# zhouxian/FluidLab

Hardware: AMD Instinct MI355X
Metric: MPM substeps/sec (fwd+bwd), 128^3 grid / 200k particles (higher is better)
Workload: dtype f32; 1 GPU; water block 128^3 grid, 200k particles (BASELINE configs[1] inputs), fwd+bwd, evolving (rolling window); nc_start=34727, nc_end=99195, parallelism=1 env, 1 GPU

## Files before the change

fluidlab_amd/csrc/fe_engine.hip:

```cpp
#include <hip/hip_runtime.h>

#include <algorithm>
#include <cstdio>
#include <cstdlib>
#include <cstring>
#include <string>
#include <vector>

#include "../../include/fluidengine.h"
#include "../../include/fluidengine_ext.h"
#include "fe_math.h"
#include "fe_grid_launch.h"

static_assert(sizeof(fe_real) == 4, "the HIP engine is fp32 (macros.py:207-211)");

#define FR_WORDS 25
#define GR_WORDS 24

template <typename T>
struct Plane {
    char* base; unsigned off;
    __host__ __device__ __forceinline__ T& operator[](int s) const { return *(T*)(base + (size_t)(off + (unsigned)s * (unsigned)sizeof(T))); }
    __host__ __device__ __forceinline__ T* ptr() const { return (T*)(base + (size_t)off); }
};
// ... 499 lines not shown
template <int NPL>
__device__ __forceinline__ void slab_store(float4* slab, int item, int l, float4 v, int wt) {
    float4* base = slab + (size_t)item * SLAB_N;
    if (NPL == 4) { if (wt) wt_store16(base, (unsigned)l * 16u, v); else base[l] = v; }
    else {
        const u32x3 u = {__float_as_uint(v.x), __float_as_uint(v.y), __float_as_uint(v.z)};
        if (wt) __builtin_amdgcn_raw_buffer_store_b96(u, wt_rsrc(base), l * 12, 0, 16);
        else __builtin_amdgcn_raw_buffer_store_b96(u, wt_rsrc(base), l * 12, 0, 0);
    }
}
__device__ __forceinline__ int tile_region(int t) { return (t + 3) >> 2; }
template <int NPL, bool SHELL_ONLY = false, bool FG = false>
__device__ __forceinline__ void tile_handover(const SimP& S, float4* slab, int item, float* acc, const GridStore& GS, const TileO& to,
                                              int nbr_entry, int l, float4 v, int wt, int& fg_d) {
    asm volatile("" : "+v"(l));
    const int tx = l >> 6, ty = (l >> 3) & 7, tz = l & 7;
    const int reg = tile_region(tx) * 9 + tile_region(ty) * 3 + tile_region(tz);
    const int e = __shfl(nbr_entry, reg, 64);
    const bool inner = ((unsigned)(tx - 1) < (unsigned)SLAB_T) & ((unsigned)(ty - 1) < (unsigned)SLAB_T) & ((unsigned)(tz - 1) < (unsigned)SLAB_T);
    if (inner) {
        if (!SHELL_ONLY) slab_store<NPL>(slab, item, ((tx - 1) * SLAB_T + (ty - 1)) * SLAB_T + (tz - 1), v, wt);
    } else if (e >= 0 && (v.x != 0.f || v.y != 0.f || v.z != 0.f || v.w != 0.f)) {
        float* dst = acc + cell_addr(to.ox + tx, to.oy + ty, to.oz + tz, S.nb);
        unsafeAtomicAdd(dst, v.x); unsafeAtomicAdd(dst + S.ncell, v.y); unsafeAtomicAdd(dst + 2 * S.ncell, v.z);
        if (NPL > 3) unsafeAtomicAdd(dst + 3 * S.ncell, v.w);
        if (FG) fg_d |= 1 << reg; else GS.dirty[e] = GS.stamp;
    }
}
template <int NPL, bool SHELL_ONLY = false>
__device__ __forceinline__ void tile_handover(const SimP& S, float4* slab, int item, float* acc, const GridStore& GS, const TileO& to,
                                              int nbr_entry, int l, float4 v, int wt) {
    int none = 0;
    tile_handover<NPL, SHELL_ONLY, false>(S, slab, item, acc, GS, to, nbr_entry, l, v, wt, none);
}

#ifndef FE_LEAN_QUADS
#define FE_LEAN_QUADS 0
#endif
__device__ __forceinline__ bool stencil_on_shell(int lb) {
    const int bx = lb >> 6, by = (lb >> 3) & 7, bz = lb & 7;
    return (bx == 0) | (bx == 5) | (by == 0) | (by == 5) | (bz == 0) | (bz == 5);
}
template <int NPL, bool FG = false>
__device__ __forceinline__ void quad_handover(const SimP& S, const int* acc, float inv_p, float inv_m, float4* slab, int item, float* accg,
                                              const GridStore& GS, const TileO& to, int nbr_entry, bool wshell, int wt, int& fg_d) {
    int lane = threadIdx.x & 63;
    asm volatile("" : "+v"(lane));
#if !FE_LEAN_QUADS
    for (int k = 0; k < TILE_N / 64; k++) {
        const int l = lane + 64 * k;
        tile_handover<NPL, false, FG>(S, slab, item, accg, GS, to, nbr_entry, l, make_float4((float)acc[l] * inv_p, (float)acc[TILE_N + l] * inv_p, (float)acc[2 * TILE_N + l] * inv_p, NPL > 3 ? (float)acc[3 * TILE_N + l] * inv_m : 0.f), wt, fg_d);
    }
    return;
#endif
#pragma unroll
    for (int k = 0; k < 4; k++) {
        const int l6 = lane + 64 * k;
        if (k < 3 || l6 < SLAB_N) {
            const int tx = l6 / 36, r = l6 - 36 * tx, ty = r / 6, tz = r - 6 * ty;
            const int l = ((tx + 1) * TILE_T + ty + 1) * TILE_T + tz + 1;
            const float4 v = make_float4((float)acc[l] * inv_p, (float)acc[TILE_N + l] * inv_p, (float)acc[2 * TILE_N + l] * inv_p, NPL > 3 ? (float)acc[3 * TILE_N + l] * inv_m : 0.f);
            slab_store<NPL>(slab, item, l6, v, wt);
        }
    }
    if (wshell) {
#pragma unroll 2
        for (int k = 0; k < TILE_N / 64; k++) {
            const int l = lane + 64 * k;
            const int tx = l >> 6, ty = (l >> 3) & 7, tz = l & 7;
            const bool inner = ((unsigned)(tx - 1) < (unsigned)SLAB_T) & ((unsigned)(ty - 1) < (unsigned)SLAB_T) & ((unsigned)(tz - 1) < (unsigned)SLAB_T);
            float4 v = make_float4(0.f, 0.f, 0.f, 0.f);
            if (!inner) v = make_float4((float)acc[l] * inv_p, (float)acc[TILE_N + l] * inv_p, (float)acc[2 * TILE_N + l] * inv_p, NPL > 3 ? (float)acc[3 * TILE_N + l] * inv_m : 0.f);
            tile_handover<NPL, true, FG>(S, slab, item, accg, GS, to, nbr_entry, l, v, wt, fg_d);
        }
    }
}
template <int NPL>
__device__ __forceinline__ void quad_handover(const SimP& S, const int* acc, float inv_p, float inv_m, float4* slab, int item, float* accg,
                                              const GridStore& GS, const TileO& to, int nbr_entry, bool wshell, int wt) {
    int none = 0;
    quad_handover<NPL, false>(S, acc, inv_p, inv_m, slab, item, accg, GS, to, nbr_entry, wshell, wt, none);
}

struct GridW {
    float* g_in; float4* slab; int ncell; int* frame_slow; int* blk_flag; int* blk_list; int* blk_count; int* err; int* slow;
    const FgDev* fg; float4* g_out;
};

__device__ __forceinline__ void carry_F(const FrameV& cur, const FrameV& nxt, m3& F) {
    if (nxt.iso == 1 && cur.iso != 1) { const float c = fe_cbrt_pos(m3_det(F)); F = m3_zero(); F.a[0][0] = F.a[1][1] = F.a[2][2] = c; }
}
__device__ __forceinline__ void unused_particle_fwd(const SimP& S, const FrameV& cur, const FrameV& nxt, int s, int pid,
                                                    const int* __restrict__ pool_idx, const AgentP& agent, const InjectP& inj, int f) {
    PState p;
    load_xvC(cur, s, p);
    load_F(cur, s, p.F);
    int used_next = 0;
    if (inj.on) {
        int j = pool_idx[pid] - inj.act_id;
        if (j >= 0 && j < inj.flux) {
            const EffP& e = agent.e[agent.inj];
            const float* rv = e.random_vector + ((size_t)inj.row * e.flux + j) * 3;
            float q[4] = {e.quat[f * 4], e.quat[f * 4 + 1], e.quat[f * 4 + 2], e.quat[f * 4 + 3]};
            float ip[3], iv[3];
            quat_rotate(e.inject_p, q, ip);
            quat_rotate(e.inject_v, q, iv);
            float vnorm = sqrtf(e.inject_v[0] * e.inject_v[0] + e.inject_v[1] * e.inject_v[1] + e.inject_v[2] * e.inject_v[2]);
#pragma unroll
            for (int d = 0; d < 3; d++) {
                float offset = (rv[d] * 2.f - 1.f) * e.radius;
                p.x[d] = offset + e.pos[f * 3 + d] + ip[d];
                p.v[d] = e.randomize_inject_v ? iv[d] + (rv[d] * 2.f - 1.f) * vnorm * 2.0f : iv[d];
            }
            used_next = 1;
        }
    }
    store_xvC(nxt, s, p.x, p.v, p.C);
    carry_F(cur, nxt, p.F);
    store_F(nxt, s, p.F);
    pstore(nxt, nxt.used, s, used_next);
}

__device__ __forceinline__ bool collector_takes(const SimP& S, const FrameV& cur, const FrameV& nxt, int s, const float4* __restrict__ info, const AgentP& agent) {
    if (agent.collector_mat >= 0 && load_info(S, info, s).mat != agent.collector_mat) return false;
    PState p;
    load_xvC(cur, s, p);
    if (!boundary_is_out(*agent.collector, p.x)) return false;
    load_F(cur, s, p.F);
    const float nowhere[3] = {-100.f, -100.f, -100.f};
    store_xvC(nxt, s, nowhere, p.v, p.C);
    carry_F(cur, nxt, p.F);
    store_F(nxt, s, p.F);
    cur.used[s] = 0; nxt.used[s] = 0;
    return true;
}

struct P2GPrep { Stencil st; float mv[3]; m3 affine; float m; bool inside; };

struct P2GRaw { PState p; PInfo info; };
__device__ __forceinline__ void p2g_load(const SimP& S, const FrameV& cur, int s, const float4* __restrict__ info_, P2GRaw& r) {
    load_xvC(cur, s, r.p);
    load_F(cur, s, r.p.F);
    r.info = load_info(S, info_, s);
}
template <bool WRITE, bool GENERAL>
__device__ __forceinline__ void p2g_compute(const SimP& S, const FrameV& nxt, int s, const P2GRaw& r, const GridW& G, P2GPrep& q, bool primary = true) {
    const PState& p = r.p;
    const PInfo& info = r.info;
    Constitutive k;
    constitutive_eval_t<GENERAL>(p.C, p.F, S.dt, info.mu, info.lam, info.mass, info.cls, S.stress_scale, k);
    if (WRITE && primary) store_F_used(nxt, s, k.Fnew, 1);
    stencil_make(p.x, S.inv_dx, q.st);
    q.inside = stencil_inside(q.st, S.n);
    if (!q.inside && primary) atomicAdd(G.err, 1);
    q.m = info.mass;
    q.affine = k.affine;
#pragma unroll
    for (int a = 0; a < 3; a++)
        q.mv[a] = q.m * p.v[a] - S.dx * (k.affine.a[a][0] * q.st.fx[0] + k.affine.a[a][1] * q.st.fx[1] + k.affine.a[a][2] * q.st.fx[2]);
}
template <bool WRITE, bool GENERAL>
__device__ __forceinline__ void p2g_prepare(const SimP& S, const FrameV& cur, const FrameV& nxt, int s,
                                            const float4* __restrict__ info_, const GridW& G, P2GPrep& q) {
    P2GRaw r;
    p2g_load(S, cur, s, info_, r);
    p2g_compute<WRITE, GENERAL>(S, nxt, s, r, G, q);
// ... 198 lines not shown
        for (int kk = 0; kk < 3; kk++) {
            const float weight = wij * st.w[kk][2];
            const float4 gv = g_out[cell_addr(st.base[0] + i, st.base[1] + j, st.base[2] + kk, S.nb)];
            const float gw[3] = {weight * gv.x, weight * gv.y, weight * gv.z};
#pragma unroll
            for (int a = 0; a < 3; a++) {
                if (kk == 0) T[a] = gw[a];
                else { T[a] = T[a] + gw[a]; Tz[a] = kk == 1 ? gw[a] : __builtin_fmaf(2.f, gw[a], Tz[a]); }
            }
        }
        const float fi = (float)i, fj = (float)j;
#pragma unroll
        for (int a = 0; a < 3; a++) {
            nv[a] = nv[a] + T[a];
            M.a[a][0] = __builtin_fmaf(fi, T[a], M.a[a][0]); M.a[a][1] = __builtin_fmaf(fj, T[a], M.a[a][1]); M.a[a][2] = M.a[a][2] + Tz[a];
        }
    }
#pragma unroll
    for (int a = 0; a < 3; a++)
#pragma unroll
        for (int b = 0; b < 3; b++) nC.a[a][b] = c4 * __builtin_fmaf(-st.fx[b], nv[a], M.a[a][b]);
}
template <bool TILE, bool ALIAS, bool ROLLED = false>
__device__ __forceinline__ void g2p_gather(const SimP& S, int lb, const Stencil& st, const float4* __restrict__ g_out, int tofs, float nv[3], m3& nC) {
    if (!TILE) { g2p_gather_global<true, ALIAS ? FE_SLOW_UNR : 1>(S, st, g_out, nv, nC); return; }
    const float* gt = ALIAS ? (const float*)s_acc : s_gtile;
    nv[0] = nv[1] = nv[2] = 0.f;
    const float c4 = 4.f * S.inv_dx;
    m3 M = m3_zero();
#pragma unroll ROLLED ? 1 : 9
    for (int ij = 0; ij < 9; ij++) {
        const int i = ij / 3, j = ij - 3 * i;
        const float wij = STW(st, i, 0) * STW(st, j, 1);
        float T[3] = {0.f, 0.f, 0.f}, Tz[3] = {0.f, 0.f, 0.f};
#pragma unroll
        for (int kk = 0; kk < 3; kk++) {
            const float weight = wij * st.w[kk][2];
            float g0, g1, g2;
            if (TILE) {
                const int l = tofs + lb + (i * TILE_T + j) * TILE_T + kk;
                g0 = gt[l]; g1 = gt[TILE_N + l]; g2 = gt[2 * TILE_N + l];
            } else {
                float4 gv = g_out[cell_addr(st.base[0] + i, st.base[1] + j, st.base[2] + kk, S.nb)];
                g0 = gv.x; g1 = gv.y; g2 = gv.z;
            }
            const float gw[3] = {weight * g0, weight * g1, weight * g2};
#pragma unroll
            for (int a = 0; a < 3; a++) { T[a] += gw[a]; if (kk > 0) Tz[a] += (float)kk * gw[a]; }
        }
#pragma unroll
        for (int a = 0; a < 3; a++) {
            nv[a] += T[a];
            M.a[a][0] += (float)i * T[a]; M.a[a][1] += (float)j * T[a]; M.a[a][2] += Tz[a];
        }
    }
#pragma unroll
    for (int a = 0; a < 3; a++)
#pragma unroll
        for (int b = 0; b < 3; b++) nC.a[a][b] = c4 * (M.a[a][b] - st.fx[b] * nv[a]);
}
template <int NIT, typename LD, typename ST>
__device__ __forceinline__ void tile_nodes_n(int t0, int nth, LD&& ld, ST&& st) {
    float4 v[NIT];
#pragma unroll
    for (int it = 0; it < NIT; it++) v[it] = ld(t0 + it * nth);
#pragma unroll
    for (int it = 0; it < NIT; it++) st(t0 + it * nth, v[it]);
}
template <bool QUADS = true, int MAXIT = 8, typename LD, typename ST>
__device__ __forceinline__ void tile_nodes(int t0, int nth, LD&& ld, ST&& st) {
    if (nth == WG) tile_nodes_n<2>(t0, nth, ld, st);
    else if (!QUADS || nth == HALF) {
        if constexpr (MAXIT >= 4) tile_nodes_n<4>(t0, nth, ld, st);
        else { tile_nodes_n<2>(t0, nth, ld, st); tile_nodes_n<2>(t0 + 2 * nth, nth, ld, st); }
    } else {
        if constexpr (MAXIT >= 8) tile_nodes_n<8>(t0, nth, ld, st);
        else if constexpr (MAXIT >= 4) { tile_nodes_n<4>(t0, nth, ld, st); tile_nodes_n<4>(t0 + 4 * nth, nth, ld, st); }
        else { for (int r = 0; r < 4; r++) tile_nodes_n<2>(t0 + 2 * r * nth, nth, ld, st); }
    }
}
__device__ __forceinline__ float4 tile_node_load(const TileO& to, const SimP& S, const float4* __restrict__ src, int l) {
    int i, j, k;
    const bool ok = tile_node(to, l, S.n, i, j, k);
    const float4 v = src[ok ? cell_addr(i, j, k, S.nb) : 0];
    return make_float4(ok ? v.x : 0.f, ok ? v.y : 0.f, ok ? v.z : 0.f, ok ? v.w : 0.f);
}
template <bool ALIAS = false>
__device__ __forceinline__ void load_tile3(const TileO& to, const SimP& S, const float4* __restrict__ src, const PairCtx& pc, int tofs_alias = 0) {
    if (!pc.live) return;
    float* gt = ALIAS ? (float*)s_acc : s_gtile;
    const int tofs = ALIAS ? tofs_alias : pc.ti * 3 * TILE_N;
    tile_nodes<ALIAS>(pc.t0, pc.nth, [&](int l) { return tile_node_load(to, S, src, l); },
                      [&](int l, const float4 v) { gt[tofs + l] = v.x; gt[tofs + TILE_N + l] = v.y; gt[tofs + 2 * TILE_N + l] = v.z; });
}

struct FuseP { float* fr_prev; const float4* g_out; int* slow; int* blk_count_prev; };
template <bool WRITE, bool GENERAL, bool FUSED = false, bool FG = false>
__device__ __forceinline__ void p2g_body(SimP S, float* fr_cur, float* fr_next, TableP T,
                                            const int* __restrict__ pool_idx, GridW G, AgentP agent, InjectP inj, int act, int f,
                                            GridStore GS, int fiso, FuseP FU = FuseP{nullptr, nullptr, nullptr, nullptr}) {
    const UnitAsk ask0 = unit_ask(T, blockIdx.x);
    const int n_slots = T.meta[5];
    HEAD_END(T.units_cap);
    if (!WRITE && GS.cap > 0 && GS.flag[f]) return;
    const int tid = threadIdx.x;
    if (WRITE && blockIdx.x == 0 && tid == 0 && act) {
        for (int i = 0; i < agent.n; i++) effector_move(agent.e[i], f);
    }
    if (FG) {
        if (blockIdx.x == 0 && tid == 0 && GS.cap > 0) __hip_atomic_store(GS.flag + f, 1, __ATOMIC_RELAXED, __HIP_MEMORY_SCOPE_AGENT);
        fg_begin(G.fg);
    }
    if (FUSED && blockIdx.x == 0 && tid == 0) *FU.blk_count_prev = 0;
    FrameV cur = frame_view(fr_cur, S.Np, 0, (!GENERAL && (fiso & 1)) ? 1 : 0);
    FrameV curw = frame_view(fr_cur, S.Np, 0);
    FrameV prev = frame_view(FUSED ? FU.fr_prev : fr_cur, S.Np);
    FrameV nxt = frame_view(fr_next, S.Np, S.wt & 1, (!GENERAL && (fiso & 2)) ? 1 : 0);
    const int slab_wt = FG ? 1 : (S.wt & 1);
    TL(S, 0);
    Unit un = unit_take(ask0);
    bool prev_quad = false;
    for (int wg = blockIdx.x; FG || wg < n_slots; wg += gridDim.x) {
        if (FG || wg != (int)blockIdx.x) un = unit_load(T, wg);
        if (FG && wg >= n_slots) break;
        if (un.a.z == -2) continue;
        if (un.a.z >= 0) {
            const PairCtx pc = unit_ctx(un);
            unit_enter(pc.quad, prev_quad);
            const int4 it = pc.it;
            const TileO to = tile_origin(it.x);
            const int aofs = pc.ti * 4 * TILE_N;
            int fg_t = 0, fg_d = 0;
            TL(S, 1);
            const int nbr_entry = neighbour_entry(T.blk_slot, S.nb, it.x);
            auto zero_tile = [&]() {
                if (pc.quad) { if (pc.live) for (int l = pc.t0; l < TILE_N; l += 64) ((int4*)((int*)s_acc + aofs))[l] = make_int4(0, 0, 0, 0); }
                else if (pc.live) for (int l = pc.t0; l < 4 * TILE_N; l += pc.nth) s_acc[aofs + l] = 0.0;
            };
            if (!FUSED) { zero_tile(); unit_sync(pc.quad); }
            FixScale fs_p = {1.f, 1.f}, fs_m = {1.f, 1.f};
            bool wshell = false;
            {
                const int wbase = pc.quad ? 0 : (pc.i & 64);
                const int cnt = __builtin_amdgcn_readfirstlane(min(64, max(0, it.z - wbase)));
                const LaneSplit ls = lane_split(cnt, (S.lsplit & 1) != 0 && !(WRITE && !FUSED && act && agent.collector));
                const int i = wbase + ls.p, s = it.y + i;
                const bool has = ls.ok && i < it.z;
                const int s_ld = has ? s : it.y;
                const int uflag = cur.used[s_ld];
                P2GRaw raw;
                if (FUSED) {
                    const int gofs_w = pc.quad ? aofs : 2 * aofs;
                    const int uprev = prev.used[s_ld];
                    const float4 a0 = prev.A0[s_ld];
                    load_F(cur, s_ld, raw.p.F);
                    raw.info = load_info(S, T.info, s_ld);
                    load_tile3<true>(to, S, FU.g_out, pc, gofs_w);
                    unit_sync(pc.quad);
                    const float xp[3] = {a0.x, a0.y, a0.z};
                    Stencil stp;
                    stencil_make(xp, S.inv_dx, stp);
                    if (has && uprev != 0 && stencil_inside(stp, S.n)) {
                        const int lbp = tile_base(to, stp);
                        if (lbp >= 0) g2p_gather<true, true>(S, lbp, stp, FU.g_out, gofs_w, raw.p.v, raw.p.C);
                        else { if (ls.primary) atomicAdd(FU.slow, 1); g2p_gather<false, true, true>(S, 0, stp, FU.g_out, 0, raw.p.v, raw.p.C); }
#pragma unroll
                        for (int a = 0; a < 3; a++) raw.p.x[a] = xp[a] + S.dt * raw.p.v[a];
                        if (ls.primary) store_xvC(curw, s, raw.p.x, raw.p.v, raw.p.C);
                    } else load_xvC(cur, s_ld, raw.p);
                    unit_sync(pc.quad);
                    zero_tile();
                    unit_sync(pc.quad);
                } else p2g_load(S, cur, s_ld, T.info, raw);
                bool used = has && uflag != 0;
                bool taken = false;
                if (WRITE && !FUSED && used && act && agent.collector) { taken = collector_takes(S, cur, nxt, s, T.info, agent); used = !taken; }
                P2GPrep q;
                q.inside = false;
                int lb = -1;
                if (used) {
                    p2g_compute<WRITE, GENERAL>(S, nxt, s, raw, G, q, ls.primary);
                    if (q.inside) lb = tile_base(to, q.st);
                } else {
                    q.m = 0.f; q.affine = m3_zero(); q.mv[0] = q.mv[1] = q.mv[2] = 0.f;
                    float zero[3] = {0.f, 0.f, 0.f};
                    stencil_make(zero, S.inv_dx, q.st);
                }
                TL(S, 2);
#ifdef FE_DUMMY_VALU
                {
                    float dmy = q.m;
#pragma unroll
                    for (int i_ = 0; i_ < FE_DUMMY_VALU; i_++) asm volatile("v_fma_f32 %0, %0, %0, %0" : "+v"(dmy));
                    asm volatile("" :: "v"(dmy));
                }
#endif
                const bool in_tile = lb >= 0;
                if (used && q.inside && !in_tile && ls.primary) { atomicAdd(G.slow, 1); p2g_scatter_global<FG>(S, q, G, GS, T.blk_slot, it.x, fg_d); }
                if (__any(in_tile)) {
                    fg_t = touch_regions<FG>(in_tile ? stencil_regions(lb) : 0, nbr_entry, GS);
                    if (pc.quad) {
                        wshell = __any(in_tile && stencil_on_shell(lb));
                        float bp = 0.f;
#pragma unroll
                        for (int a = 0; a < 3; a++) bp = fmaxf(bp, fabsf(q.mv[a]) + 2.f * S.dx * (fabsf(q.affine.a[a][0]) + fabsf(q.affine.a[a][1]) + fabsf(q.affine.a[a][2])));
                        fs_p = fix_scale(wave_max(in_tile ? bp : 0.f));
                        fs_m = fix_scale(wave_max(in_tile ? q.m : 0.f));
                        if (__any(in_tile && !(bp <= 3.4e38f))) fs_p.inv = __int_as_float(0x7fc00000);
                        const float sp = in_tile ? fs_p.s : 1.f;
                        q.m *= in_tile ? fs_m.s : 1.f;
#pragma unroll
                        for (int a = 0; a < 3; a++) { q.mv[a] *= sp; q.affine.a[a][0] *= sp; q.affine.a[a][1] *= sp; q.affine.a[a][2] *= sp; }
                        p2g_scatter_tile_split<true>(S, q, in_tile, in_tile ? lb : 0, aofs, ls);
                    } else p2g_scatter_tile_split<false>(S, q, in_tile, in_tile ? lb : 0, aofs, ls);
                }
                if (has && !used && !taken && WRITE && ls.primary) unused_particle_fwd(S, cur, nxt, s, T.pid_of_slot[s], pool_idx, agent, inj, f);
            }
            TL(S, 4);
            unit_sync(pc.quad);
            TL(S, 5);
            if (pc.quad) {
                if (pc.live) quad_handover<4, FG>(S, (const int*)s_acc + aofs, fs_p.inv, fs_m.inv, G.slab, pc.slab, G.g_in, GS, to, nbr_entry, wshell, slab_wt, fg_d);
            } else if (pc.live) for (int l = pc.t0; l < TILE_N; l += pc.nth)
                tile_handover<4, false, FG>(S, G.slab, pc.slab, G.g_in, GS, to, nbr_entry, l,
                                 make_float4((float)s_acc[aofs + l], (float)s_acc[aofs + TILE_N + l], (float)s_acc[aofs + 2 * TILE_N + l], (float)s_acc[aofs + 3 * TILE_N + l]), slab_wt, fg_d);
            if (FG) fg_unit_end(T, pc, nbr_entry, fg_t, fg_d);
            else unit_sync(pc.quad);
            TL(S, 6);
        } else {
            const int s = un.a.y + tid;
            if (s < S.N) {
                P2GRaw raw;
                bool have = false;
                if (FUSED && prev.used[s]) {
                    const float4 a0 = prev.A0[s];
                    const float xp[3] = {a0.x, a0.y, a0.z};
                    Stencil stp;
                    stencil_make(xp, S.inv_dx, stp);
                    if (stencil_inside(stp, S.n)) {
                        g2p_gather<false, true, true>(S, 0, stp, FU.g_out, 0, raw.p.v, raw.p.C);
#pragma unroll
                        for (int a = 0; a < 3; a++) raw.p.x[a] = xp[a] + S.dt * raw.p.v[a];
                        store_xvC(curw, s, raw.p.x, raw.p.v, raw.p.C);
                        have = true;
                    }
                }
                if (cur.used[s]) {
                    if (WRITE && !FUSED && act && agent.collector && collector_takes(S, cur, nxt, s, T.info, agent)) continue;
                    P2GPrep q;
                    if (FUSED && have) { load_F(cur, s, raw.p.F); raw.info = load_info(S, T.info, s); p2g_compute<WRITE, GENERAL>(S, nxt, s, raw, G, q); }
                    else p2g_prepare<WRITE, GENERAL>(S, cur, nxt, s, T.info, G, q);
                    int none = 0;
                    if (q.inside) p2g_scatter_global<FG>(S, q, G, GS, T.blk_slot, -1, none);
                } else if (WRITE) unused_particle_fwd(S, cur, nxt, s, T.pid_of_slot[s], pool_idx, agent, inj, f);
            }
        }
    }
}
struct P2GArgs { SimP S; float* fr_cur; float* fr_next; TableP T; const int* pool_idx; GridW G; AgentP agent; InjectP inj; int act; int f; GridStore GS; int fiso; FuseP FU; };
template <bool WRITE, bool GENERAL>
__global__ FE_KALIGN __launch_bounds__(WG, GENERAL ? 3 : 4) void k_p2g(const UnitRec* h_units, const int* h_meta, int h_cap, SimP S, float* fr_cur, float* fr_next, TableP T, const int* pool_idx, GridW G, AgentP agent, InjectP inj, int act, int f, GridStore GS, int fiso) { T.units = h_units; T.meta = h_meta; T.units_cap = h_cap; p2g_body<WRITE, GENERAL>(S, fr_cur, fr_next, T, pool_idx, G, agent, inj, act, f, GS, fiso); }
template <bool GENERAL>
__global__ FE_KALIGN __launch_bounds__(WG, GENERAL ? 3 : 4) void k_g2p_p2g(const UnitRec* h_units, const int* h_meta, int h_cap, SimP S, float* fr_cur, float* fr_next, TableP T, const int* pool_idx, GridW G, AgentP agent, InjectP inj, int act, int f, GridStore GS, int fiso, FuseP FU) { T.units = h_units; T.meta = h_meta; T.units_cap = h_cap; p2g_body<true, GENERAL, true>(S, fr_cur, fr_next, T, pool_idx, G, agent, inj, act, f, GS, fiso, FU); }
template <typename ARGS>
__device__ __forceinline__ const ARGS* fg_args_again() {
    const ARGS* p = (const ARGS*)__builtin_amdgcn_kernarg_segment_ptr();
    asm volatile("" : "+s"(p));
    return p;
}
template <bool GENERAL>
__global__ FE_KALIGN __launch_bounds__(WG, GENERAL ? 3 : 4) void k_p2g_fg(P2GArgs A) {
    p2g_body<true, GENERAL, false, true>(A.S, A.fr_cur, A.fr_next, A.T, A.pool_idx, A.G, A.agent, A.inj, A.act, A.f, A.GS, A.fiso);
    const P2GArgs* B = fg_args_again<P2GArgs>();
    TL(B->S, 3);
    fg_owner_phase<false>(B->S, B->T, B->GS, FgArgs{B->G.fg, B->G.slab, B->G.g_in, B->G.g_out, B->G.blk_list, B->G.blk_count, B->G.blk_flag, B->f});
}
template <bool GENERAL>
__global__ FE_KALIGN __launch_bounds__(WG, GENERAL ? 3 : 4) void k_g2p_p2g_fg(P2GArgs A) {
    p2g_body<true, GENERAL, true, true>(A.S, A.fr_cur, A.fr_next, A.T, A.pool_idx, A.G, A.agent, A.inj, A.act, A.f, A.GS, A.fiso, A.FU);
    const P2GArgs* B = fg_args_again<P2GArgs>();
    TL(B->S, 3);
    fg_owner_phase<false>(B->S, B->T, B->GS, FgArgs{B->G.fg, B->G.slab, B->G.g_in, B->G.g_out, B->G.blk_list, B->G.blk_count, B->G.blk_flag, B->f});
}
template <bool GENERAL>
__global__ FE_KALIGN __launch_bounds__(WG, GENERAL ? 3 : 4) void k_g2p_p2g_b(Batch<P2GArgs> B) { const P2GArgs& A = B.a[blockIdx.y]; p2g_body<true, GENERAL, true>(A.S, A.fr_cur, A.fr_next, A.T, A.pool_idx, A.G, A.agent, A.inj, A.act, A.f, A.GS, A.fiso, A.FU); }
template <bool WRITE, bool GENERAL>
__global__ FE_KALIGN __launch_bounds__(WG, GENERAL ? 3 : 4) void k_p2g_b(Batch<P2GArgs> B) { const P2GArgs& A = B.a[blockIdx.y]; p2g_body<WRITE, GENERAL>(A.S, A.fr_cur, A.fr_next, A.T, A.pool_idx, A.G, A.agent, A.inj, A.act, A.f, A.GS, A.fiso); }


template <bool NODE>
__device__ __forceinline__ bool agent_collide_particle(const SimP& S, const AgentP& agent, int f, const float x[3], float nv[3]) {
    const float sdt = NODE ? 0.f : S.dt;
    bool any = false;
    for (int ei = 0; ei < agent.n; ei++) {
        const EffP& e = agent.e[ei];
        if (!e.has_mesh) continue;
        const float pos[3] = {x[0] + sdt * nv[0], x[1] + sdt * nv[1], x[2] + sdt * nv[2]};
        if (!(pos[1] > agent.collide_min_y)) continue;
        float out[3];
        any |= t_dynamic_collide<float>(e.mesh, e.pos + f * 3, e.quat + f * 4, e.pos + (f + 1) * 3, e.quat + (f + 1) * 4, pos, nv, S.dt, out);
        nv[0] = out[0]; nv[1] = out[1]; nv[2] = out[2];
    }
    return any;
}
#define FE_MAX_STATICS 4
struct NodeWork { int c, ni, nj, nk; float4 gi; float go[3]; float pad; };
struct StaticsP { int n; const SdfP* s; };

// ... 1593 lines not shown
            __syncthreads();
            TL(S, 4);
        } else {
            if (QLIST) unit_enter(false, prev_quad);
            const int s = un.a.y + tid;
            TileO none = {0, 0, 0};
            P2GRaw none_pre;
            if (s < S.N) slot_p2g_grad<false, GENERAL, false>(S, cur, Gn, Gc, s, T, pool_idx, none, gg_in, slow, agent, inj, f, 0, 0, none_pre, D);
        }
    }
}
struct P2GGradArgs { SimP S; float* fr_cur; float* Gn_; float* Gc_; TableP T; const int* pool_idx; const float4* gg_in; int* blk_count; int* slow; AgentP agent; InjectP inj; int act; int f; float* Gd_; const int* to_slot; int fiso; };
template <bool GENERAL, int MINW>
__global__ FE_KALIGN __launch_bounds__(WG, MINW) void k_p2g_grad(const UnitRec* h_units, const UnitRec* h_units_p, const int* h_meta, int h_cap, SimP S, float* fr_cur, float* Gn_, float* Gc_, TableP T, const int* pool_idx, const float4* gg_in, int* blk_count, int* slow, AgentP agent, InjectP inj, int act, int f, float* Gd_, const int* to_slot, int fiso) { T.units = h_units; T.units_p = h_units_p; T.meta = h_meta; T.units_cap = h_cap; p2g_grad_body<GENERAL, MINW>(S, fr_cur, Gn_, Gc_, T, pool_idx, gg_in, blk_count, slow, agent, inj, act, f, Gd_, to_slot, fiso); }
template <bool GENERAL, int MINW>
__global__ FE_KALIGN __launch_bounds__(WG, MINW) void k_p2g_grad_b(Batch<P2GGradArgs> B) { const P2GGradArgs& A = B.a[blockIdx.y]; p2g_grad_body<GENERAL, MINW>(A.S, A.fr_cur, A.Gn_, A.Gc_, A.T, A.pool_idx, A.gg_in, A.blk_count, A.slow, A.agent, A.inj, A.act, A.f, A.Gd_, A.to_slot, A.fiso); }

struct BwdFuseP { float* fr_prev; float* Gp_; const float4* g_out; float* gg_out; float4* slab; };
template <int MINW, bool GENERAL = false>
__device__ __forceinline__ void p2g_grad_g2p_grad_body(SimP S, float* fr_cur, float* Gn_, float* Gc_, TableP T, const int* __restrict__ pool_idx,
                                                         const float4* __restrict__ gg_in, int* blk_count, int* slow, AgentP agent, InjectP inj, int act, int f,
                                                         int fiso, BwdFuseP B, GridStore GS) {
    const UnitAsk ask0 = unit_ask<GENERAL>(T, blockIdx.x);
    const int n_slots = T.meta[GENERAL ? 9 : 5];
    HEAD_END(T.units_cap);
    const Unit un0 = unit_take(ask0);
    const int tid = threadIdx.x;
    if (blockIdx.x == 0 && tid == 0) {
        *blk_count = 0;
        if (act) for (int i = agent.n - 1; i >= 0; i--) effector_move_grad(agent.e[i], f);
    }
    VoutSrc V; V.g_out = B.g_out; V.store = GS.data + (size_t)(f - 1) * GS.cap * GS_BLK; V.blk_slot = T.blk_slot;
    constexpr int AR = GENERAL ? 2 : 1;
    FrameV cur = frame_view(fr_cur, S.Np, 0, (!GENERAL && (fiso & 1)) ? 1 : 0), prev = frame_view(B.fr_prev, S.Np);
    FrameV Gn = frame_view(Gn_, S.Np, 0, (!GENERAL && (fiso & 2)) ? 2 : 0);
    FrameV Gc = frame_view(Gc_, S.Np, S.wt & 8, (!GENERAL && (fiso & 4)) ? 2 : 0);
    FrameV Gp = frame_view(B.Gp_, S.Np, S.wt & 4);
    const GradDst D = {Gc, nullptr, T.pid_of_slot};
    float* const t4 = lds_tile4<AR>();
    double* const acc3 = lds_acc3<AR>();
    bool prev_quad = false, any_tail = false;
    for (int wg = blockIdx.x; ; wg += gridDim.x) {
        Unit un = un0;
        if (wg != (int)blockIdx.x) un = unit_load<GENERAL>(T, wg);
        if (wg >= n_slots) break;
        if (un.a.z == -2) continue;
        if (un.a.z >= 0) {
            const PairCtx pc = GENERAL ? pair_ctx(un) : unit_ctx(un);
            unit_enter(pc.quad, prev_quad);
            const int4 it = pc.it;
            const TileO to = tile_origin(it.x);
            const int wbase = pc.quad ? 0 : (pc.i & 64);
            const int cnt = __builtin_amdgcn_readfirstlane(min(64, max(0, it.z - wbase)));
            const LaneSplit ls = lane_split(cnt, false);
            const int i = wbase + ls.p;
            const bool has = ls.ok && i < it.z;
            const int s = it.y + (has ? i : 0);
            const int nbr_entry = neighbour_entry(T.blk_slot, S.nb, it.x);
            float* tl = t4 + pc.ti * 4 * TILE_N;
            if (pc.live) tile_nodes<!GENERAL>(pc.t0, pc.nth, [&](int l) { return tile_node_load(to, S, gg_in, l); },
                                              [&](int l, const float4 v) { tl[l] = v.x; tl[TILE_N + l] = v.y; tl[2 * TILE_N + l] = v.z; tl[3 * TILE_N + l] = v.w; });
            unit_sync(pc.quad);
            PState g;
            bool kept = false;
            P2GRaw no_pre;
            if (has) {
                if (pc.quad) kept = slot_p2g_grad<true, GENERAL, false, true, 1, AR, true>(S, cur, Gn, Gc, s, T, pool_idx, to, gg_in, slow, agent, inj, f, 0, 0, no_pre, D, tl, 0, ls.primary, &g);
                else kept = slot_p2g_grad<true, GENERAL, false, false, 1, AR, true>(S, cur, Gn, Gc, s, T, pool_idx, to, gg_in, slow, agent, inj, f, pc.ti * 4 * TILE_N, 0, no_pre, D, nullptr, 0, ls.primary, &g);
            }
            if (!kept) {
#pragma unroll
                for (int a = 0; a < 3; a++) { g.x[a] = 0.f; g.v[a] = 0.f; }
                g.C = m3_zero();
            }
            asm volatile("" : "+v"(g.x[0]), "+v"(g.x[1]), "+v"(g.x[2]), "+v"(g.v[0]), "+v"(g.v[1]), "+v"(g.v[2]));
            asm volatile("" : "+v"(g.C.a[0][0]), "+v"(g.C.a[0][1]), "+v"(g.C.a[0][2]), "+v"(g.C.a[1][0]), "+v"(g.C.a[1][1]), "+v"(g.C.a[1][2]), "+v"(g.C.a[2][0]), "+v"(g.C.a[2][1]), "+v"(g.C.a[2][2]));
            unit_sync(pc.quad);
            const int tofs = pc.quad ? pc.ti * 4 * TILE_N - 6 * TILE_N : pc.ti * 3 * TILE_N;
            const int u0 = prev.used[s];
            const float4 a00 = prev.A0[s];
            float* gt = pc.quad ? (float*)acc3 + tofs : lds_tile3<AR>() + tofs;
            g2p_grad_load_tile2<!GENERAL, GENERAL ? 2 : 4>(to, S, B.g_out, V.store, nbr_entry, pc, gt);
            if (!pc.quad && pc.live) for (int l = pc.t0; l < 3 * TILE_N; l += pc.nth) acc3[tofs + l] = 0.0;
            unit_sync(pc.quad);
            float inv = 1.f;
            bool wshell = false;
            {
                const bool used = has && u0 != 0;
                float x[3] = {0.f, 0.f, 0.f};
                if (used) { x[0] = a00.x; x[1] = a00.y; x[2] = a00.z; }
                Stencil st;
                stencil_make(x, S.inv_dx, st);
                const bool inside = used && stencil_inside(st, S.n);
                const int lb = inside ? tile_base(to, st) : -1;
                const bool live = lb >= 0;
                if (has && kept && ls.primary && !inside) store_xvC(Gc, s, g.x, g.v, g.C);
                if (pc.quad) wshell = __any(live && stencil_on_shell(lb));
                if (__any(live)) {
                    if (pc.quad) inv = g2p_grad_particle2<4, true, 1, AR>(S, Gc, Gp, s, live ? lb : 0, st, live, tofs, gt, 0, true, &g);
                    else g2p_grad_particle2<4, false, 1, AR>(S, Gc, Gp, s, live ? lb : 0, st, live, tofs, gt, 0, true, &g);
                } else if (pc.quad && pc.live) {
                    asm volatile("s_waitcnt lgkmcnt(0)" ::: "memory");
                    for (int l = pc.t0; l < 3 * TILE_N; l += pc.nth) ((int*)acc3)[tofs + l] = 0;
                }
                g2p_grad_wave_slow<true>(S, Gc, Gp, s, a00, inside && !live && ls.primary, used && !inside && ls.primary, V, B.gg_out, slow, GS, &g, it.x, nbr_entry);
            }
            unit_sync(pc.quad);
            if (pc.quad) {
                if (pc.live) quad_handover<3>(S, (const int*)acc3 + tofs, inv, inv, B.slab, pc.slab, B.gg_out, GS, to, nbr_entry, wshell, S.wt & 4);
            } else if (pc.live) for (int l = pc.t0; l < TILE_N; l += pc.nth)
                tile_handover<3>(S, B.slab, pc.slab, B.gg_out, GS, to, nbr_entry, l,
                                 make_float4((float)acc3[tofs + l], (float)acc3[tofs + TILE_N + l], (float)acc3[tofs + 2 * TILE_N + l], 0.f), S.wt & 4);
            unit_sync(pc.quad);
        } else any_tail = true;
    }
    if (!any_tail) return;
    __syncthreads();
    for (int wg = blockIdx.x; wg < n_slots; wg += gridDim.x) {
        const Unit un = unit_load<GENERAL>(T, wg);
        if (un.a.z != -1) continue;
        {
            int t_ = tid;
            asm volatile("" : "+v"(t_));
            const int s = un.a.y + t_;
            TileO none = {0, 0, 0};
            P2GRaw none_pre;
            if (s < S.N) {
                PState g;
                const bool kept = slot_p2g_grad<false, GENERAL, false, false, 1, AR, true>(S, cur, Gn, Gc, s, T, pool_idx, none, gg_in, slow, agent, inj, f, 0, 0, none_pre, D, nullptr, 0, true, &g);
                if (kept) {
                    if (!prev.used[s]) store_xvC(Gc, s, g.x, g.v, g.C);
                    else g2p_grad_slot_global<true>(S, prev, Gc, Gp, s, V, B.gg_out, agent, f - 1, GS, &g);
                }
            }
        }
    }
}
struct PggArgs { SimP S; float* fr_cur; float* Gn_; float* Gc_; TableP T; const int* pool_idx; const float4* gg_in; int* blk_count; int* slow; AgentP agent; InjectP inj; int act; int f; int fiso; BwdFuseP B; GridStore GS; };
#ifndef FE_FB_WAVES_LESS
#define FE_FB_WAVES_LESS 0
#endif
template <int MINW, bool GENERAL = false>
__global__ FE_KALIGN __launch_bounds__(WG, MINW - FE_FB_WAVES_LESS) void k_pgg_g2pg(const UnitRec* h_list, const int* h_meta, int h_cap, SimP S, float* fr_cur, float* Gn_, float* Gc_, TableP T, const int* pool_idx, const float4* gg_in, int* blk_count, int* slow, AgentP agent, InjectP inj, int act, int f, int fiso, BwdFuseP B, GridStore GS) { if (GENERAL) T.units_p = h_list; else T.units = h_list; T.meta = h_meta; T.units_cap = h_cap; p2g_grad_g2p_grad_body<MINW, GENERAL>(S, fr_cur, Gn_, Gc_, T, pool_idx, gg_in, blk_count, slow, agent, inj, act, f, fiso, B, GS); }
template <int MINW>
__global__ FE_KALIGN __launch_bounds__(WG, MINW - FE_FB_WAVES_LESS) void k_pgg_g2pg_b(Batch<PggArgs> Bt) { const PggArgs& A = Bt.a[blockIdx.y]; p2g_grad_g2p_grad_body<MINW>(A.S, A.fr_cur, A.Gn_, A.Gc_, A.T, A.pool_idx, A.gg_in, A.blk_count, A.slow, A.agent, A.inj, A.act, A.f, A.fiso, A.B, A.GS); }


#ifndef SORT_YFAST
#define SORT_YFAST 0
#endif
#define SORT_HB 4096
__device__ __forceinline__ int row_iscan(int x) {
    x += __builtin_amdgcn_update_dpp(0, x, 0x111, 0xf, 0xf, false);
    x += __builtin_amdgcn_update_dpp(0, x, 0x112, 0xf, 0xf, false);
    x += __builtin_amdgcn_update_dpp(0, x, 0x114, 0xf, 0xf, false);
    x += __builtin_amdgcn_update_dpp(0, x, 0x118, 0xf, 0xf, false);
    return x;
}
__device__ __forceinline__ int wave_iscan(int x) {
    x = row_iscan(x);
    x += __builtin_amdgcn_update_dpp(0, x, 0x142, 0xa, 0xf, false);
    x += __builtin_amdgcn_update_dpp(0, x, 0x143, 0xc, 0xf, false);
    return x;
}
__global__ __launch_bounds__(256) void k_sort_count(SimP S, float* fr, int n_pwg, int* key, int* rank, int* cnt, int* bcnt,
                                                    const int* __restrict__ clr_active, const int* __restrict__ clr_meta, int* clr_slot, int* nact) {
    __shared__ int hist[SORT_HB + 1];
    __shared__ int kmin;
    const int tid = threadIdx.x;
    if (blockIdx.x == 0 && tid == 0) *nact = 0;
    if ((int)blockIdx.x >= n_pwg) {
        const int n = clr_meta[2];
        for (int i = (blockIdx.x - n_pwg) * 256 + tid; i < n; i += SORT_CLR_WGS * 256) clr_slot[clr_active[i]] = -1;
        return;
    }
    const int s = blockIdx.x * blockDim.x + tid;
    const bool valid = s < S.N;
    int kk = S.ncell;
    if (valid) {
        FrameV cur = frame_view(fr, S.Np);
        const float4 a0 = cur.A0[s];
        if (cur.used[s]) {
            float x[3] = {a0.x, a0.y, a0.z};
            Stencil st;
            stencil_make(x, S.inv_dx, st);
            if (stencil_inside(st, S.n)) {
                kk = cell_addr(st.base[0], st.base[1], st.base[2], S.nb);
#if SORT_YFAST
                kk = (kk & ~63) | ((st.base[0] & 3) << 4) | ((st.base[2] & 3) << 2) | (st.base[1] & 3);
#endif
            }
        }
    }
    const bool is_tail = kk == S.ncell;
    if (tid == 0) kmin = 0x7fffffff;
// ... 2655 lines not shown
```

Before: 12070 substep_pairs/s.

## Skip shell handover in pair tiles when no particle touches the tile shell

```diff
diff --git a/fluidlab_amd/csrc/fe_engine.hip b/fluidlab_amd/csrc/fe_engine.hip
--- a/fluidlab_amd/csrc/fe_engine.hip
+++ b/fluidlab_amd/csrc/fe_engine.hip
@@ -605,6 +605,37 @@
     quad_handover<NPL, false>(S, acc, inv_p, inv_m, slab, item, accg, GS, to, nbr_entry, wshell, wt, none);
 }
 
+__shared__ int s_shell[2];
+__device__ __forceinline__ void pair_shell_clear(const PairCtx& pc) {
+    if (pc.quad) return;
+    int t = pc.t0;
+    asm volatile("" : "+v"(t));
+    if (t == 0) s_shell[pc.ti] = 0;
+}
+__device__ __forceinline__ void pair_shell_mark(const PairCtx& pc, bool wshell) {
+    if (pc.quad || !wshell) return;
+    int lane = threadIdx.x & 63;
+    asm volatile("" : "+v"(lane));
+    if (lane == 0) s_shell[pc.ti] = 1;
+}
+template <int NPL, bool FG = false, typename RD>
+__device__ __forceinline__ void pair_handover(const SimP& S, float4* slab, const PairCtx& pc, float* accg, const GridStore& GS, const TileO& to,
+                                              int nbr_entry, RD&& rd, int wt, int& fg_d) {
+    int t = pc.t0;
+    asm volatile("" : "+v"(t));
+#pragma unroll 1
+    for (int r = 0; r < TILE_N; r += 2 * pc.nth) {
+        const int l6 = t + (r >> 1);
+        if (l6 < SLAB_N) {
+            const int tx = (l6 * 57) >> 11, q = l6 - 36 * tx, ty = (q * 43) >> 8, tz = q - 6 * ty;
+            slab_store<NPL>(slab, pc.slab, l6, rd(((tx + 1) * TILE_T + ty + 1) * TILE_T + tz + 1), wt);
+        }
+    }
+    if (__builtin_amdgcn_readfirstlane(s_shell[pc.ti])) {
+        for (int l = pc.t0; l < TILE_N; l += pc.nth) tile_handover<NPL, true, FG>(S, slab, pc.slab, accg, GS, to, nbr_entry, l, rd(l), wt, fg_d);
+    }
+}
+
 struct GridW {
     float* g_in; float4* slab; int ncell; int* frame_slow; int* blk_flag; int* blk_list; int* blk_count; int* err; int* slow;
     const FgDev* fg; float4* g_out;
@@ -969,7 +1000,8 @@
 __device__ __forceinline__ float4 tile_node_load(const TileO& to, const SimP& S, const float4* __restrict__ src, int l) {
     int i, j, k;
     const bool ok = tile_node(to, l, S.n, i, j, k);
-    const float4 v = src[ok ? cell_addr(i, j, k, S.nb) : 0];
+    const int a = (((i >> 2) * (S.nb * S.nb * 64)) | ((i & 3) << 4)) + (((((j >> 2) * S.nb) + (k >> 2)) << 6) | ((j & 3) << 2) | (k & 3));
+    const float4 v = src[ok ? a : 0];
     return make_float4(ok ? v.x : 0.f, ok ? v.y : 0.f, ok ? v.z : 0.f, ok ? v.w : 0.f);
 }
 template <bool ALIAS = false>
@@ -1023,6 +1055,7 @@
             auto zero_tile = [&]() {
                 if (pc.quad) { if (pc.live) for (int l = pc.t0; l < TILE_N; l += 64) ((int4*)((int*)s_acc + aofs))[l] = make_int4(0, 0, 0, 0); }
                 else if (pc.live) for (int l = pc.t0; l < 4 * TILE_N; l += pc.nth) s_acc[aofs + l] = 0.0;
+                pair_shell_clear(pc);
             };
             if (!FUSED) { zero_tile(); unit_sync(pc.quad); }
             FixScale fs_p = {1.f, 1.f}, fs_m = {1.f, 1.f};
@@ -1099,7 +1132,10 @@
 #pragma unroll
                         for (int a = 0; a < 3; a++) { q.mv[a] *= sp; q.affine.a[a][0] *= sp; q.affine.a[a][1] *= sp; q.affine.a[a][2] *= sp; }
                         p2g_scatter_tile_split<true>(S, q, in_tile, in_tile ? lb : 0, aofs, ls);
-                    } else p2g_scatter_tile_split<false>(S, q, in_tile, in_tile ? lb : 0, aofs, ls);
+                    } else {
+                        pair_shell_mark(pc, __any(in_tile && stencil_on_shell(lb)));
+                        p2g_scatter_tile_split<false>(S, q, in_tile, in_tile ? lb : 0, aofs, ls);
+                    }
                 }
                 if (has && !used && !taken && WRITE && ls.primary) unused_particle_fwd(S, cur, nxt, s, T.pid_of_slot[s], pool_idx, agent, inj, f);
             }
@@ -1108,9 +1144,8 @@
             TL(S, 5);
             if (pc.quad) {
                 if (pc.live) quad_handover<4, FG>(S, (const int*)s_acc + aofs, fs_p.inv, fs_m.inv, G.slab, pc.slab, G.g_in, GS, to, nbr_entry, wshell, slab_wt, fg_d);
-            } else if (pc.live) for (int l = pc.t0; l < TILE_N; l += pc.nth)
-                tile_handover<4, false, FG>(S, G.slab, pc.slab, G.g_in, GS, to, nbr_entry, l,
-                                 make_float4((float)s_acc[aofs + l], (float)s_acc[aofs + TILE_N + l], (float)s_acc[aofs + 2 * TILE_N + l], (float)s_acc[aofs + 3 * TILE_N + l]), slab_wt, fg_d);
+            } else if (pc.live) pair_handover<4, FG>(S, G.slab, pc, G.g_in, GS, to, nbr_entry, [&](int l) {
+                return make_float4((float)s_acc[aofs + l], (float)s_acc[aofs + TILE_N + l], (float)s_acc[aofs + 2 * TILE_N + l], (float)s_acc[aofs + 3 * TILE_N + l]); }, slab_wt, fg_d);
             if (FG) fg_unit_end(T, pc, nbr_entry, fg_t, fg_d);
             else unit_sync(pc.quad);
             TL(S, 6);
@@ -2870,6 +2905,7 @@
             float* gt = pc.quad ? (float*)acc3 + tofs : lds_tile3<AR>() + tofs;
             g2p_grad_load_tile2<!GENERAL, GENERAL ? 2 : 4>(to, S, B.g_out, V.store, nbr_entry, pc, gt);
             if (!pc.quad && pc.live) for (int l = pc.t0; l < 3 * TILE_N; l += pc.nth) acc3[tofs + l] = 0.0;
+            pair_shell_clear(pc);
             unit_sync(pc.quad);
             float inv = 1.f;
             bool wshell = false;
@@ -2884,6 +2920,7 @@
                 const bool live = lb >= 0;
                 if (has && kept && ls.primary && !inside) store_xvC(Gc, s, g.x, g.v, g.C);
                 if (pc.quad) wshell = __any(live && stencil_on_shell(lb));
+                else pair_shell_mark(pc, __any(live && stencil_on_shell(lb)));
                 if (__any(live)) {
                     if (pc.quad) inv = g2p_grad_particle2<4, true, 1, AR>(S, Gc, Gp, s, live ? lb : 0, st, live, tofs, gt, 0, true, &g);
                     else g2p_grad_particle2<4, false, 1, AR>(S, Gc, Gp, s, live ? lb : 0, st, live, tofs, gt, 0, true, &g);
@@ -2896,9 +2933,8 @@
             unit_sync(pc.quad);
             if (pc.quad) {
                 if (pc.live) quad_handover<3>(S, (const int*)acc3 + tofs, inv, inv, B.slab, pc.slab, B.gg_out, GS, to, nbr_entry, wshell, S.wt & 4);
-            } else if (pc.live) for (int l = pc.t0; l < TILE_N; l += pc.nth)
-                tile_handover<3>(S, B.slab, pc.slab, B.gg_out, GS, to, nbr_entry, l,
-                                 make_float4((float)acc3[tofs + l], (float)acc3[tofs + TILE_N + l], (float)acc3[tofs + 2 * TILE_N + l], 0.f), S.wt & 4);
+            } else if (pc.live) { int none = 0; pair_handover<3>(S, B.slab, pc, B.gg_out, GS, to, nbr_entry, [&](int l) {
+                return make_float4((float)acc3[tofs + l], (float)acc3[tofs + TILE_N + l], (float)acc3[tofs + 2 * TILE_N + l], 0.f); }, S.wt & 4, none); }
             unit_sync(pc.quad);
         } else any_tail = true;
     }
```

After: 11890 substep_pairs/s. 1.5% lower.
